# anshium/visual-place-recognition-and-geopose-estimation

Hardware: AMD Instinct MI355X
Metric: images/sec end-to-end (backbone->SALAD->kNN->pose) (higher is better)
Workload: dtype bf16; 1 GPU; DINOv2 vit_large/14 (random init) + SALAD + bf16 kNN k=10 over a 100000-row x 8448 synthetic gallery sharded 1 way(s) + fused (lat,lon,sin,cos) head; 3x224x224 bf16 images; batch_per_gpu=64, global_batch=64, gallery_rows=100000, k=10, parallelism=dp1+gallery-shard1, batches_in_flight=1, graph_retrieval=False

## Files before the change

visual-place-recognition-and-geopose-estimation_amd/csrc/attention.hip:

```cpp
#include <stdlib.h>
#include "vpr_common.h"
#include "vpr_internal.h"

namespace vpr {

constexpr int AT_D = 64;
constexpr int AT_KP = 288;


__device__ __forceinline__ int vtile_off(int row, int chunk) { return row * 128 + ((chunk ^ (row & 7)) << 4); }

struct AttnCtx {
  const char* Ks; const char* Vs; const uint16_t* qb; long long tok_stride; int T, qcol, g, trq, trp;
  float scale_log2e; uint16_t* out; long long out_stride;
  long long row_base, tail_base; int Tp;
};
__device__ __forceinline__ long long attn_row(const AttnCtx& cx, int t) {
  return t < cx.Tp ? cx.row_base + t : cx.tail_base + (t - cx.Tp);
}
typedef __attribute__((ext_vector_type(4))) short s16x4;

__device__ __forceinline__ void attn_load_q(const AttnCtx& cx, int qt, bf16x8 (&bq)[2]) {
  const int qrow = min(qt * 16 + cx.qcol, cx.T - 1);
#pragma unroll
  for (int s = 0; s < 2; ++s)
    bq[s] = *reinterpret_cast<const bf16x8*>(cx.qb + attn_row(cx, qrow) * cx.tok_stride + 32 * s + 8 * cx.g);
}
__device__ __forceinline__ f32x4 attn_qk_block(const AttnCtx& cx, int kb, const bf16x8 (&bq)[2]) {
  f32x4 acc = {0.f, 0.f, 0.f, 0.f};
#pragma unroll
  for (int s = 0; s < 2; ++s)
    acc = __builtin_amdgcn_mfma_f32_16x16x32_bf16(lds_frag(cx.Ks, 16 * kb + cx.qcol, cx.g + 4 * s), bq[s], acc, 0, 0, 0);
  return acc;
}
__device__ __forceinline__ void attn_qk_all(const AttnCtx& cx, const bf16x8 (&bq)[2], f32x4 (&sc)[AT_KP / 16]) {
#pragma unroll
  for (int kb = 0; kb < AT_KP / 16; ++kb) {
    sc[kb] = attn_qk_block(cx, kb, bq);
    if ((kb % 3) == 2) __builtin_amdgcn_sched_barrier(0);
  }
}
__device__ __forceinline__ void attn_mask_block(f32x4& s, int kb, int klast, int lim) {
  if (kb > klast) {
    asm volatile("");
    s = f32x4{-INFINITY, -INFINITY, -INFINITY, -INFINITY};
  } else if (kb == klast) {
    asm volatile("");
#pragma unroll
    for (int e = 0; e < 4; ++e) s[e] = e < lim ? s[e] : -INFINITY;
  }
}
__device__ __forceinline__ float attn_rowmax(const AttnCtx& cx, f32x4 (&sc)[AT_KP / 16]) {
  const int klast = (cx.T - 1) >> 4;
  const int lim = cx.T - 16 * klast - 4 * cx.g;
  if (klast < AT_KP / 16 - 2) {
#pragma unroll
    for (int kb = 0; kb < AT_KP / 16 - 2; ++kb) attn_mask_block(sc[kb], kb, klast, lim);
  }
#pragma unroll
  for (int kb = AT_KP / 16 - 2; kb < AT_KP / 16; ++kb) attn_mask_block(sc[kb], kb, klast, lim);
  float mx = sc[0][0];
#pragma unroll
  for (int kb = 0; kb < AT_KP / 16; ++kb) {
    mx = fmaxf(fmaxf(mx, sc[kb][0]), sc[kb][1]);
    mx = fmaxf(fmaxf(mx, sc[kb][2]), sc[kb][3]);
  }
  mx = fmaxf(mx, __shfl_xor(mx, 16, 64));
  return fmaxf(mx, __shfl_xor(mx, 32, 64));
}
__device__ __forceinline__ void attn_phase1(const AttnCtx& cx, f32x4 (&sc)[AT_KP / 16], float mx,
                                             bf16x8 (&pb)[AT_KP / 32], bool has_next, const bf16x8 (&bq)[2]) {
  const float nm = -mx * cx.scale_log2e;
#pragma unroll
  for (int t = 0; t < AT_KP / 32; ++t) {
    float p[8];
#pragma unroll
    for (int e = 0; e < 4; ++e) {
      p[e] = __builtin_amdgcn_exp2f(fmaf(sc[2 * t][e], cx.scale_log2e, nm));
      p[4 + e] = __builtin_amdgcn_exp2f(fmaf(sc[2 * t + 1][e], cx.scale_log2e, nm));
    }
    if (has_next) {
      sc[2 * t] = attn_qk_block(cx, 2 * t, bq);
      sc[2 * t + 1] = attn_qk_block(cx, 2 * t + 1, bq);
    }
#pragma unroll
    for (int j = 0; j < 8; ++j) pb[t][j] = (__bf16)p[j];
  }
}
__device__ __forceinline__ float attn_phase2(const AttnCtx& cx, const bf16x8 (&pb)[AT_KP / 32], int qt, bool has_next, f32x4 (&sn)[AT_KP / 16]) {
  const bf16x8 ones = {(__bf16)1.f, (__bf16)1.f, (__bf16)1.f, (__bf16)1.f, (__bf16)1.f, (__bf16)1.f, (__bf16)1.f, (__bf16)1.f};
  f32x4 sacc = {0.f, 0.f, 0.f, 0.f};
#pragma unroll
  for (int t = 0; t < AT_KP / 32; ++t) sacc = __builtin_amdgcn_mfma_f32_16x16x32_bf16(ones, pb[t], sacc, 0, 0, 0);
  f32x4 oacc[4];
#pragma unroll
  for (int db = 0; db < 4; ++db) {
    oacc[db] = f32x4{0.f, 0.f, 0.f, 0.f};
#pragma unroll
    for (int t = 0; t < AT_KP / 32; ++t) {
      const int r0 = 32 * t + 4 * cx.g + cx.trq;
      const s16x4 lo = __builtin_amdgcn_ds_read_tr16_b64_v4i16(
          (__attribute__((address_space(3))) s16x4*)(cx.Vs + vtile_off(r0, 2 * db + (cx.trp >> 1)) + 8 * (cx.trp & 1)));
      const s16x4 hi = __builtin_amdgcn_ds_read_tr16_b64_v4i16(
          (__attribute__((address_space(3))) s16x4*)(cx.Vs + vtile_off(r0 + 16, 2 * db + (cx.trp >> 1)) + 8 * (cx.trp & 1)));
      const s16x8 av = {lo[0], lo[1], lo[2], lo[3], hi[0], hi[1], hi[2], hi[3]};
      oacc[db] = __builtin_amdgcn_mfma_f32_16x16x32_bf16(__builtin_bit_cast(bf16x8, av), pb[t], oacc[db], 0, 0, 0);
      if ((t % 3) == 2) __builtin_amdgcn_sched_barrier(0);
    }
  }
  const float inv = 1.0f / sacc[0];
  float mxn = 0.f;
  if (has_next) mxn = attn_rowmax(cx, sn);
  const int q = qt * 16 + cx.qcol;
  if (q < cx.T) {
    uint16_t* orow = cx.out + attn_row(cx, q) * cx.out_stride;
#pragma unroll
    for (int db = 0; db < 4; ++db) {
      ushort4 o;
      o.x = f32_to_bf16_bits(oacc[db][0] * inv);
      o.y = f32_to_bf16_bits(oacc[db][1] * inv);
      o.z = f32_to_bf16_bits(oacc[db][2] * inv);
      o.w = f32_to_bf16_bits(oacc[db][3] * inv);
      *reinterpret_cast<ushort4*>(orow + 16 * db + 4 * cx.g) = o;
    }
  }
  return mxn;
}

template <int NW, bool PIPE, int ABL = 0>
__global__ __launch_bounds__(NW * 64, NW / 2) void attention_kernel(
    const uint16_t* __restrict__ qkv, uint16_t* __restrict__ out, int T, int Tp, long long tail_row0, int H,
    float scale_log2e, int dephase) {
  extern __shared__ __attribute__((aligned(16))) char smem[];
  if (dephase > 0 && blockIdx.x >= 256 && blockIdx.x < 512)
    for (int i = 0; i < dephase; ++i) __builtin_amdgcn_s_sleep(33);
  char* Ks = smem;
  char* Vs = smem + AT_KP * 128;
  const int bh = blockIdx.x, b = bh / H, h = bh % H;
  const int tid = threadIdx.x, lane = tid & 63, wave = tid >> 6;
  const long long tok_stride = 3LL * H * AT_D;
  const uint16_t* qb = qkv + (long long)h * AT_D;
  const uint16_t* kb_ = qb + (long long)H * AT_D;
  const uint16_t* vb = qb + 2LL * H * AT_D;

  constexpr int NT = NW * 64;
  constexpr int AT_MAXT = (AT_KP / 16 + NW - 1) / NW;
  bf16x8 qf[AT_MAXT][2];
  {
    AttnCtx c0;
    c0.qb = qb; c0.tok_stride = tok_stride; c0.T = T; c0.qcol = lane & 15; c0.g = lane >> 4;
    c0.Tp = Tp; c0.row_base = (long long)b * Tp; c0.tail_base = tail_row0 + (long long)b * (T - Tp);
#pragma unroll
    for (int j = 0; j < AT_MAXT; ++j) attn_load_q(c0, min(wave + NW * j, ((T + 15) >> 4) - 1), qf[j]);
  }
  constexpr int NLD = (AT_KP * 8 + NT - 1) / NT;
  s16x8 kreg[NLD], vreg[NLD];
#pragma unroll
  for (int it = 0; it < NLD; ++it) {
    const int i = min(tid + NT * it, AT_KP * 8 - 1);
    const int key = i >> 3, ch = i & 7;
    const int kc = key < T ? key : T - 1;
    const long long krow = kc < Tp ? (long long)b * Tp + kc : tail_row0 + (long long)b * (T - Tp) + (kc - Tp);
    kreg[it] = *reinterpret_cast<const s16x8*>(kb_ + krow * tok_stride + ch * 8);
    vreg[it] = *reinterpret_cast<const s16x8*>(vb + krow * tok_stride + ch * 8);
  }
#pragma unroll
  for (int it = 0; it < NLD; ++it) {
    const int i = min(tid + NT * it, AT_KP * 8 - 1);
    const int key = i >> 3, ch = i & 7;
    const s16x8 z = {0, 0, 0, 0, 0, 0, 0, 0};
    const s16x8 kv = key < T ? kreg[it] : z, vv = key < T ? vreg[it] : z;
    *reinterpret_cast<s16x8*>(Ks + tile_off(key, ch)) = kv;
    *reinterpret_cast<s16x8*>(Vs + vtile_off(key, ch)) = vv;
  }
  __syncthreads();

  if (ABL == 3) return;
  const int qcol = lane & 15, g = lane >> 4;
  const int ntile = (T + 15) >> 4;

  AttnCtx cx;
  cx.Ks = Ks; cx.Vs = Vs; cx.qb = qb; cx.tok_stride = tok_stride; cx.T = T; cx.qcol = qcol; cx.g = g;
  cx.trq = (lane & 15) >> 2; cx.trp = lane & 3; cx.scale_log2e = scale_log2e;
  cx.out = out + (long long)h * AT_D; cx.out_stride = (long long)H * AT_D;
  cx.Tp = Tp; cx.row_base = (long long)b * Tp; cx.tail_base = tail_row0 + (long long)b * (T - Tp);

  f32x4 sc[AT_KP / 16];
  bf16x8 pb[AT_KP / 32];
  if (wave >= ntile) return;
  if constexpr (PIPE) {
    attn_qk_all(cx, qf[0], sc);
    float mx = attn_rowmax(cx, sc);
#pragma unroll
    for (int j = 0; j < AT_MAXT; ++j) {
      const int qt = wave + NW * j;
      if (qt < ntile) {
        const bool has_next = qt + NW < ntile;
        attn_phase1(cx, sc, mx, pb, has_next, qf[j + 1 < AT_MAXT ? j + 1 : j]);
        mx = attn_phase2(cx, pb, qt, has_next, sc);
      }
    }
  } else {
#pragma unroll
    for (int j = 0; j < AT_MAXT; ++j) {
      const int qt = wave + NW * j;
      if (qt < ntile) {
        attn_qk_all(cx, qf[j], sc);
        if (ABL == 4) {
          float a = 0.f;
#pragma unroll
          for (int kb = 0; kb < AT_KP / 16; ++kb) a += sc[kb][0] + sc[kb][1] + sc[kb][2] + sc[kb][3];
          if (qt * 16 + cx.qcol < T) cx.out[attn_row(cx, qt * 16 + cx.qcol) * cx.out_stride + 4 * cx.g] = f32_to_bf16_bits(a);
          continue;
        }
        const float mx = attn_rowmax(cx, sc);
        attn_phase1(cx, sc, mx, pb, false, qf[j]);
        if (ABL == 2) {
          float a = 0.f;
#pragma unroll
          for (int t = 0; t < AT_KP / 32; ++t)
#pragma unroll
            for (int e = 0; e < 8; ++e) a += (float)pb[t][e];
          if (qt * 16 + cx.qcol < T) cx.out[attn_row(cx, qt * 16 + cx.qcol) * cx.out_stride + 4 * cx.g] = f32_to_bf16_bits(a);
          continue;
        }
        attn_phase2(cx, pb, qt, false, sc);
      }
    }
  }
}

constexpr size_t AT_LDS = (size_t)2 * AT_KP * 128;

}

using namespace vpr;

static int attention_launch(const uint16_t* qkv, uint16_t* out, int B, int T, int Tp, long long tail_row0, int H,
                            int head_dim, float scale, void* stream) {
  if (!qkv || !out || B <= 0 || T <= 0 || H <= 0 || Tp < 0 || Tp > T || tail_row0 < 0) return VPR_ERR_INVALID_ARG;
  if (!(scale > 0.f && scale <= 3.4e38f)) return VPR_ERR_INVALID_ARG;
  if (head_dim != AT_D || T > AT_KP || (long long)B * H > 0x7fffffffLL) return VPR_ERR_UNSUPPORTED;
  if ((reinterpret_cast<uintptr_t>(qkv) | reinterpret_cast<uintptr_t>(out)) & 15) return VPR_ERR_UNSUPPORTED;
  const int variant = tune_or(TUNE_ATTN_VARIANT, 0);
  const float c = scale * 1.4426950408889634f;
  const int dephase = (variant >= 20 && variant <= 60) ? variant - 20 : 0;
  hipStream_t st = static_cast<hipStream_t>(stream);
#define VPR_ATTN_LAUNCH(NW, PIPE)                                                                        \
  do {                                                                                                   \
    VPR_TRY_LAUNCH((launch_kernel_lds<attention_kernel<NW, PIPE>>(dim3((unsigned)(B * H)), dim3(NW * 64), AT_LDS, st, \
                                                                  qkv, out, T, Tp, tail_row0, H, c, dephase)));     \
  } while (0)
#ifdef VPR_ABLATION
#define VPR_ATTN_ABL(A)                                                                                   \
  do {                                                                                                   \
    VPR_TRY_LAUNCH((launch_kernel_lds<attention_kernel<8, false, A>>(dim3((unsigned)(B * H)), dim3(512), AT_LDS, st, \
                                                                     qkv, out, T, Tp, tail_row0, H, c, 0)));        \
  } while (0)
#endif
  switch (variant) {
    case 1: VPR_ATTN_LAUNCH(4, false); break;
    case 2: VPR_ATTN_LAUNCH(4, true); break;
    case 3: VPR_ATTN_LAUNCH(6, false); break;
#ifdef VPR_ABLATION
    case 12: VPR_ATTN_ABL(2); break;
    case 13: VPR_ATTN_ABL(3); break;
    case 14: VPR_ATTN_ABL(4); break;
#endif
    default: VPR_ATTN_LAUNCH(8, false); break;
  }
#undef VPR_ATTN_LAUNCH
#ifdef VPR_ABLATION
#undef VPR_ATTN_ABL
#endif
  return VPR_OK;
}

extern "C" int vpr_attention_qkv_bf16(const uint16_t* qkv, uint16_t* out, int B, int T, int H, int head_dim,
                                      float scale, void* stream) {
  return attention_launch(qkv, out, B, T, T, 0, H, head_dim, scale, stream);
}

extern "C" int vpr_attention_qkv_split_bf16(const uint16_t* qkv, uint16_t* out, int B, int T, int body_tokens,
                                            long long tail_row0, int H, int head_dim, float scale, void* stream) {
  return attention_launch(qkv, out, B, T, body_tokens, tail_row0, H, head_dim, scale, stream);
}
```

visual-place-recognition-and-geopose-estimation_amd/csrc/backbone_rows.h:

```cpp
#pragma once
#include <initializer_list>
#include "vpr_common.h"
#include "vpr_internal.h"

namespace vpr {


template <int NCH>
__device__ __forceinline__ void ln_load_row(const uint16_t* x, const uint16_t* res, uint16_t* sum_out, const float* pre_bias,
                                            long long off, bool store_sum, int nchunks, int lane, float (&v)[NCH][8], float& s) {
  s = 0.f;
#pragma unroll
  for (int i = 0; i < NCH; ++i) {
    const int ch = lane + 64 * i;
    if (ch < nchunks) {
      const s16x8 q = *reinterpret_cast<const s16x8*>(x + off + ch * 8);
      if (res != nullptr) {
        const s16x8 r = *reinterpret_cast<const s16x8*>(res + off + ch * 8);
        s16x8 o;
#pragma unroll
        for (int e = 0; e < 8; ++e) {
          const uint16_t sb = f32_to_bf16_bits(bf16_bits_to_f32((uint16_t)q[e]) + bf16_bits_to_f32((uint16_t)r[e]));
          o[e] = (short)sb;
          v[i][e] = bf16_bits_to_f32(sb);
          s += v[i][e];
        }
        if (store_sum) *reinterpret_cast<s16x8*>(sum_out + off + ch * 8) = o;
      } else if (pre_bias != nullptr) {
        const float4 p0 = *reinterpret_cast<const float4*>(pre_bias + ch * 8);
        const float4 p1 = *reinterpret_cast<const float4*>(pre_bias + ch * 8 + 4);
        const float pb[8] = {p0.x, p0.y, p0.z, p0.w, p1.x, p1.y, p1.z, p1.w};
#pragma unroll
        for (int e = 0; e < 8; ++e) { v[i][e] = bf16_bits_to_f32((uint16_t)q[e]) + pb[e]; s += v[i][e]; }
      } else {
#pragma unroll
        for (int e = 0; e < 8; ++e) { v[i][e] = bf16_bits_to_f32((uint16_t)q[e]); s += v[i][e]; }
      }
    } else {
#pragma unroll
      for (int e = 0; e < 8; ++e) v[i][e] = 0.f;
    }
  }
}

template <int NCH>
__device__ __forceinline__ void ln_stats(const float (&v)[NCH][8], float s, int C, float eps, int lane, float& mean, float& rstd) {
  mean = wave_sum(s) / (float)C;
  float ss = 0.f;
#pragma unroll
  for (int i = 0; i < NCH; ++i)
    if (lane + 64 * i < (C >> 3)) {
#pragma unroll
      for (int e = 0; e < 8; ++e) { const float d = v[i][e] - mean; ss = fmaf(d, d, ss); }
    }
  rstd = 1.0f / sqrtf(wave_sum(ss) / (float)C + eps);
}

template <typename ParamT>
__device__ __forceinline__ float ln_param(const ParamT* p, int ch, int e) {
  if constexpr (sizeof(ParamT) == 16) return bf16_bits_to_f32((uint16_t)p[ch][e]);
  else if constexpr (sizeof(ParamT) == 2) return bf16_bits_to_f32((uint16_t)p[ch * 8 + e]);
  else return p[ch * 8 + e];
}

template <int NCH, typename ParamT>
__device__ __forceinline__ void ln_store_row(const float (&v)[NCH][8], float mean, float rstd, const ParamT* gamma,
                                             const ParamT* beta, uint16_t* y, long long off, int nchunks, int lane) {
#pragma unroll
  for (int i = 0; i < NCH; ++i) {
    const int ch = lane + 64 * i;
    if (ch < nchunks) {
      s16x8 o;
#pragma unroll
      for (int e = 0; e < 8; ++e) {
        const float g = ln_param(gamma, ch, e), b = ln_param(beta, ch, e);
        o[e] = (short)f32_to_bf16_bits((v[i][e] - mean) * rstd * g + b);
      }
      *reinterpret_cast<s16x8*>(y + off + ch * 8) = o;
    }
  }
}


template <int MBW, bool QUAD = false>
struct SkinnyOperands {
  const uint16_t* wp;
  const uint16_t* ip[MBW];
  __device__ __forceinline__ SkinnyOperands(const uint16_t* W, int ldw, int n0, int N, const uint16_t* in, long long ldi, int m0,
                                            int M, int lane) {
    const int r = QUAD ? lane >> 2 : lane & 15, g = QUAD ? lane & 3 : lane >> 4;
    wp = W + (long long)min(n0 + r, N - 1) * ldw + 8 * g;
#pragma unroll
    for (int mb = 0; mb < MBW; ++mb) ip[mb] = in + (long long)min(m0 + mb * 16 + r, M - 1) * ldi + 8 * g;
  }
};

__device__ __forceinline__ bf16x8 skinny_to_mfma_lane(bf16x8 f) {
  typedef __attribute__((ext_vector_type(4))) int i32x4;
  const int src = 4 * (4 * (int)(threadIdx.x & 15) + (int)((threadIdx.x & 63) >> 4));
  i32x4 v = __builtin_bit_cast(i32x4, f);
#pragma unroll
  for (int e = 0; e < 4; ++e) v[e] = __builtin_amdgcn_ds_bpermute(src, v[e]);
  return __builtin_bit_cast(bf16x8, v);
}

template <int UNR, int MBW, bool QUAD>
__device__ __forceinline__ void skinny_k_slice(const SkinnyOperands<MBW, QUAD>& o, int kbeg, int kend, f32x4 (&acc)[MBW]) {
  const auto frag = [](const uint16_t* p) -> bf16x8 {
    const bf16x8 f = *reinterpret_cast<const bf16x8*>(p);
    if constexpr (QUAD) return skinny_to_mfma_lane(f); else return f;
  };
  f32x4 a[MBW];
#pragma unroll
  for (int mb = 0; mb < MBW; ++mb) a[mb] = f32x4{0.f, 0.f, 0.f, 0.f};
  int ks = kbeg;
  for (; ks + UNR <= kend; ks += UNR) {
    bf16x8 wf[UNR], xf[UNR][MBW];
#pragma unroll
    for (int u = 0; u < UNR; ++u) {
      wf[u] = frag(o.wp + (ks + u) * 32);
#pragma unroll
      for (int mb = 0; mb < MBW; ++mb) xf[u][mb] = frag(o.ip[mb] + (ks + u) * 32);
    }
#pragma unroll
    for (int u = 0; u < UNR; ++u)
#pragma unroll
      for (int mb = 0; mb < MBW; ++mb) a[mb] = __builtin_amdgcn_mfma_f32_16x16x32_bf16(wf[u], xf[u][mb], a[mb], 0, 0, 0);
  }
  for (; ks < kend; ++ks) {
    const bf16x8 wf = frag(o.wp + ks * 32);
#pragma unroll
    for (int mb = 0; mb < MBW; ++mb)
      a[mb] = __builtin_amdgcn_mfma_f32_16x16x32_bf16(wf, frag(o.ip[mb] + ks * 32), a[mb], 0, 0, 0);
  }
#pragma unroll
  for (int mb = 0; mb < MBW; ++mb) acc[mb] = a[mb];
}

template <int NW, int MBW>
__device__ __forceinline__ bool skinny_reduce(const f32x4 (&acc)[MBW], float (&red)[NW][MBW][64][4], int lane, int wave, f32x4& s) {
#pragma unroll
  for (int mb = 0; mb < MBW; ++mb) *reinterpret_cast<f32x4*>(&red[wave][mb][lane][0]) = acc[mb];
  __syncthreads();
  if (NW > MBW && wave >= MBW) return false;
  s = *reinterpret_cast<const f32x4*>(&red[0][wave][lane][0]);
#pragma unroll
  for (int p = 1; p < NW; ++p) {
    const f32x4 t = *reinterpret_cast<const f32x4*>(&red[p][wave][lane][0]);
    s[0] += t[0]; s[1] += t[1]; s[2] += t[2]; s[3] += t[3];
  }
  return true;
}

__device__ __forceinline__ void skinny_store4(uint16_t* op, const uint16_t (&ob)[4], int n, int N, int ldo) {
  if (n + 3 < N && (ldo & 3) == 0) {
    ushort4 o;
    o.x = ob[0]; o.y = ob[1]; o.z = ob[2]; o.w = ob[3];
    *reinterpret_cast<ushort4*>(op) = o;
  } else {
    for (int e = 0; e < 4 && n + e < N; ++e) op[e] = ob[e];
  }
}

__device__ __forceinline__ float gelu_tanh(float x) {
  const float u = 0.7978845608028654f * x * fmaf(0.044715f * x, x, 1.0f);
  return x / (1.0f + __expf(-2.0f * u));
}


__device__ __forceinline__ void row_stats_write16(float* __restrict__ row_stats, int p, int m, int M, const uint16_t (&ob)[4],
                                                  const float* __restrict__ stats_bias, int n, int N, int lane) {
  float t[4];
#pragma unroll
  for (int e = 0; e < 4; ++e)
    t[e] = bf16_bits_to_f32(ob[e]) + (stats_bias != nullptr && n + e < N ? stats_bias[n + e] : 0.f);
  float sm = (t[0] + t[1]) + (t[2] + t[3]);
  sm += __shfl_xor(sm, 16, 64);
  sm += __shfl_xor(sm, 32, 64);
  const float mean = sm * (1.0f / 16.0f);
  float m2 = 0.f;
#pragma unroll
  for (int e = 0; e < 4; ++e) { const float d = t[e] - mean; m2 = fmaf(d, d, m2); }
  m2 += __shfl_xor(m2, 16, 64);
  m2 += __shfl_xor(m2, 32, 64);
  if ((lane >> 4) == 0 && m < M) {
    float* dst = row_stats + ((long long)p * M + m) * 2;
    dst[0] = mean; dst[1] = m2;
  }
}

__device__ __forceinline__ void row_stats_merge(const float* __restrict__ row_stats, int P, int M, int row, int part, float& mean,
                                                float& m2) {
  const float* ps = row_stats + (long long)row * 2;
  const long long pstride = (long long)M * 2;
  float sm = 0.f;
#pragma unroll 8
  for (int p = part; p < P; p += 4) sm += ps[p * pstride];
  sm += __shfl_xor(sm, 1, 64);
  sm += __shfl_xor(sm, 2, 64);
  mean = sm / (float)P;
  m2 = 0.f;
#pragma unroll 8
  for (int p = part; p < P; p += 4) {
    const float2 q = *reinterpret_cast<const float2*>(ps + p * pstride);
    const float d = q.x - mean;
    m2 += q.y + 16.0f * d * d;
  }
  m2 += __shfl_xor(m2, 1, 64);
  m2 += __shfl_xor(m2, 2, 64);
}

inline bool ln_shape_ok(long long M, int C) { return (C % 8) == 0 && C <= 2048 && M <= 0x1fffffffcLL; }

inline int ln_check(std::initializer_list<const void*> chunked, const void* gamma, const void* beta, long long M, int C) {
  for (const void* p : chunked)
    if (!p) return VPR_ERR_INVALID_ARG;
  if (!gamma || !beta || M < 0 || C <= 0) return VPR_ERR_INVALID_ARG;
  if (M == 0) return VPR_OK;
  if (!ln_shape_ok(M, C)) return VPR_ERR_UNSUPPORTED;
  for (const void* p : chunked)
    if (!aligned16(p)) return VPR_ERR_UNSUPPORTED;
  return VPR_OK;
}

template <typename F>
inline int ln_dispatch_nch(int C, F&& f) {
  switch ((C / 8 + 63) / 64) {
    case 1: return f(std::integral_constant<int, 1>{});
    case 2: return f(std::integral_constant<int, 2>{});
    case 3: return f(std::integral_constant<int, 3>{});
    case 4: return f(std::integral_constant<int, 4>{});
    default: return VPR_ERR_UNSUPPORTED;
  }
}

}
```

visual-place-recognition-and-geopose-estimation_amd/csrc/layernorm.hip:

```cpp
#include "backbone_rows.h"

namespace vpr {

template <int NCH, typename ParamT, int RW>
__global__ __launch_bounds__(256) void layernorm_bf16_kernel(
    const uint16_t* __restrict__ x, const uint16_t* __restrict__ res, uint16_t* __restrict__ sum_out,
    const float* __restrict__ pre_bias, const ParamT* __restrict__ gamma, const ParamT* __restrict__ beta,
    float eps, uint16_t* __restrict__ y, long long M, int C) {
  static_assert(RW == 1 || RW == 2, "one or two rows per wave");
  const int lane = threadIdx.x & 63, wave = threadIdx.x >> 6;
  const long long row0 = ((long long)blockIdx.x * 4 + wave) * RW;
  if (row0 >= M) return;
  const int nchunks = C >> 3;
  const bool second = RW == 2 && row0 + 1 < M;
  float v[RW][NCH][8], s[RW], mean, rstd;
  ln_load_row<NCH>(x, res, sum_out, pre_bias, row0 * C, true, nchunks, lane, v[0], s[0]);
  if constexpr (RW == 2)
    ln_load_row<NCH>(x, res, sum_out, pre_bias, (second ? row0 + 1 : M - 1) * C, second, nchunks, lane, v[1], s[1]);
  ln_stats<NCH>(v[0], s[0], C, eps, lane, mean, rstd);
  ln_store_row<NCH>(v[0], mean, rstd, gamma, beta, y, row0 * C, nchunks, lane);
  if constexpr (RW == 2) {
    if (!second) return;
    ln_stats<NCH>(v[1], s[1], C, eps, lane, mean, rstd);
    ln_store_row<NCH>(v[1], mean, rstd, gamma, beta, y, (row0 + 1) * C, nchunks, lane);
  }
}

template <typename ParamT>
static int launch_ln(const uint16_t* x, const uint16_t* res, uint16_t* sum_out, const float* pb, const ParamT* g, const ParamT* b,
                     float eps, uint16_t* y, long long M, int C, hipStream_t stream) {
  const int rw = tune_or(TUNE_LN_ROWS, 1);
  return ln_dispatch_nch(C, [&](auto nch) {
    constexpr int NCH = decltype(nch)::value;
    if constexpr (NCH <= 2)
      if (rw == 2)
        return launch_kernel(layernorm_bf16_kernel<NCH, ParamT, 2>, dim3((unsigned)((M + 7) / 8)), dim3(256), 0, stream,
                             x, res, sum_out, pb, g, b, eps, y, M, C);
    return launch_kernel(layernorm_bf16_kernel<NCH, ParamT, 1>, dim3((unsigned)((M + 3) / 4)), dim3(256), 0, stream,
                         x, res, sum_out, pb, g, b, eps, y, M, C);
  });
}

static int ln_entry(std::initializer_list<const void*> chunked, const uint16_t* x, const uint16_t* res, uint16_t* sum_out,
                    const float* pb, const void* gamma, const void* beta, int params_are_bf16, float eps, uint16_t* y,
                    long long M, int C, void* stream) {
  const int st = ln_check(chunked, gamma, beta, M, C);
  if (st != VPR_OK || M == 0) return st;
  hipStream_t s = static_cast<hipStream_t>(stream);
  if (params_are_bf16)
    return launch_ln(x, res, sum_out, pb, static_cast<const uint16_t*>(gamma), static_cast<const uint16_t*>(beta), eps, y, M, C, s);
  return launch_ln(x, res, sum_out, pb, static_cast<const float*>(gamma), static_cast<const float*>(beta), eps, y, M, C, s);
}

}

using namespace vpr;

extern "C" int vpr_layernorm_bf16(const uint16_t* x, const void* gamma, const void* beta, int params_are_bf16,
                                  float eps, uint16_t* y, long long M, int C, void* stream) {
  return ln_entry({x, y}, x, nullptr, nullptr, nullptr, gamma, beta, params_are_bf16, eps, y, M, C, stream);
}

extern "C" int vpr_add_layernorm_bf16(const uint16_t* x, const uint16_t* res, uint16_t* sum_out, const void* gamma,
                                      const void* beta, int params_are_bf16, float eps, uint16_t* y, long long M,
                                      int C, void* stream) {
  return ln_entry({x, y, res, sum_out}, x, res, sum_out, nullptr, gamma, beta, params_are_bf16, eps, y, M, C, stream);
}

extern "C" int vpr_bias_layernorm_bf16(const uint16_t* x, const float* pre_bias, const void* gamma, const void* beta,
                                       int params_are_bf16, float eps, uint16_t* y, long long M, int C, void* stream) {
  return ln_entry({x, y, pre_bias}, x, nullptr, nullptr, pre_bias, gamma, beta, params_are_bf16, eps, y, M, C, stream);
}
```

visual-place-recognition-and-geopose-estimation_amd/csrc/vpr_common.h:

```cpp
#pragma once
#include <hip/hip_runtime.h>
#include <stdint.h>

namespace vpr {

typedef __attribute__((ext_vector_type(8))) short s16x8;
typedef __attribute__((ext_vector_type(8))) __bf16 bf16x8;
typedef __attribute__((ext_vector_type(4))) float f32x4;
typedef __attribute__((ext_vector_type(16))) float f32x16;
typedef __attribute__((ext_vector_type(4))) int i32x4;
typedef __attribute__((ext_vector_type(8))) int i32x8;

constexpr int WAVE = 64;

__device__ __forceinline__ long long vpr_clock_now() {
  unsigned long long t;
  asm volatile("s_memrealtime %0\n\ts_waitcnt lgkmcnt(0)" : "=s"(t) : : "memory");
  return (long long)t;
}

__device__ __forceinline__ float bf16_bits_to_f32(uint16_t v) {
  return __uint_as_float(((uint32_t)v) << 16);
}
__device__ __forceinline__ uint16_t f32_to_bf16_bits(float f) {
  __bf16 h = (__bf16)f;
  return __builtin_bit_cast(uint16_t, h);
}

__device__ __forceinline__ void split_hi_lo(float v, uint16_t& hi, uint16_t& lo) {
  hi = f32_to_bf16_bits(v);
  lo = f32_to_bf16_bits(v - bf16_bits_to_f32(hi));
}

__device__ __forceinline__ void lds_barrier() {
  asm volatile("s_waitcnt lgkmcnt(0)" ::: "memory");
  __builtin_amdgcn_s_barrier();
}

__device__ __forceinline__ float wave_sum(float v) {
#pragma unroll
  for (int o = 32; o > 0; o >>= 1) v += __shfl_xor(v, o, 64);
  return v;
}
__device__ __forceinline__ float wave_max(float v) {
#pragma unroll
  for (int o = 32; o > 0; o >>= 1) v = fmaxf(v, __shfl_xor(v, o, 64));
  return v;
}
__device__ __forceinline__ double wave_sum_f64(double v) {
#pragma unroll
  for (int o = 32; o > 0; o >>= 1) v += __shfl_xor(v, o, 64);
  return v;
}

template <int CTRL>
__device__ __forceinline__ float dpp_f32(float v) {
  return __builtin_bit_cast(float, __builtin_amdgcn_update_dpp(0, __builtin_bit_cast(int, v), CTRL, 0xf, 0xf, true));
}
__device__ __forceinline__ float row16_max(float v) {
  v = fmaxf(v, dpp_f32<0xB1>(v));
  v = fmaxf(v, dpp_f32<0x4E>(v));
  v = fmaxf(v, dpp_f32<0x141>(v));
  v = fmaxf(v, dpp_f32<0x140>(v));
  return v;
}
__device__ __forceinline__ float row16_sum(float v) {
  v += dpp_f32<0xB1>(v);
  v += dpp_f32<0x4E>(v);
  v += dpp_f32<0x141>(v);
  v += dpp_f32<0x140>(v);
  return v;
}

__device__ __forceinline__ uint32_t f32_orderable(float f) {
  const uint32_t u = __float_as_uint(f);
  return (u & 0x80000000u) ? ~u : (u | 0x80000000u);
}
__device__ __forceinline__ float f32_from_orderable(uint32_t o) {
  const uint32_t u = (o & 0x80000000u) ? (o & 0x7fffffffu) : ~o;
  return __uint_as_float(u);
}
__device__ __forceinline__ unsigned long long make_key(float v, int idx) {
  return ((unsigned long long)f32_orderable(v) << 32) | (uint32_t)(0x7fffffff - idx);
}
__device__ __forceinline__ int key_idx(unsigned long long k) { return 0x7fffffff - (int)(uint32_t)k; }
__device__ __forceinline__ float key_val(unsigned long long k) { return f32_from_orderable((uint32_t)(k >> 32)); }

constexpr unsigned long long KEY_DEAD = 0ull;

__device__ __forceinline__ unsigned long long candidate_key(float val, int id, bool in_range) {
  return (in_range && id >= 0) ? make_key(val, id) : KEY_DEAD;
}
__device__ __forceinline__ void store_entry(unsigned long long k, float* __restrict__ out_val,
                                            int32_t* __restrict__ out_idx, long long o, int index_base = 0) {
  out_val[o] = k == KEY_DEAD ? -INFINITY : key_val(k);
  out_idx[o] = k == KEY_DEAD ? -1 : key_idx(k) + index_base;
}

constexpr int TILE_ROW_BYTES = 128;
__device__ __forceinline__ int tile_off(int row, int chunk) {
  return row * TILE_ROW_BYTES + ((chunk ^ ((row >> 1) & 7)) << 4);
}
__device__ __forceinline__ int stage_src_off(int tr, int lane) {
  return ((lane & 7) ^ ((tr >> 1) & 7)) << 4;
}

template <int AUX = 0>
__device__ __forceinline__ void glds16(const void* gsrc, void* lds_wave_base) {
  __builtin_amdgcn_global_load_lds(
      (const __attribute__((address_space(1))) void*)gsrc,
      (__attribute__((address_space(3))) void*)lds_wave_base, 16, 0, AUX);
}

__device__ __forceinline__ bf16x8 lds_frag(const char* tile, int row, int chunk) {
  return *reinterpret_cast<const bf16x8*>(tile + tile_off(row, chunk));
}

template <typename Chunk>
__device__ __forceinline__ i32x8 e4m3_operand(Chunk lo, Chunk hi) {
  const i32x4 l = __builtin_bit_cast(i32x4, lo), h = __builtin_bit_cast(i32x4, hi);
  return i32x8{l[0], l[1], l[2], l[3], h[0], h[1], h[2], h[3]};
}
constexpr int E8M0_ONE = 127;
__device__ __forceinline__ f32x4 mfma_e4m3_16x16x128(i32x8 a, i32x8 b, f32x4 c) {
  return __builtin_amdgcn_mfma_scale_f32_16x16x128_f8f6f4(a, b, c, 0, 0, 0, E8M0_ONE, 0, E8M0_ONE);
}
__device__ __forceinline__ f32x16 mfma_e4m3_32x32x64(i32x8 a, i32x8 b, f32x16 c) {
  return __builtin_amdgcn_mfma_scale_f32_32x32x64_f8f6f4(a, b, c, 0, 0, 0, E8M0_ONE, 0, E8M0_ONE);
}

__device__ __forceinline__ int xcd_tile(int orig, int nwg) {
  const int xcd = orig & 7, q = nwg >> 3, r = nwg & 7;
  return (xcd < r ? xcd * (q + 1) : r * (q + 1) + (xcd - r) * q) + (orig >> 3);
}

__device__ __forceinline__ uint4 philox4x32_10(uint4 c, uint32_t k0, uint32_t k1) {
#pragma unroll
  for (int r = 0; r < 10; ++r) {
    const uint32_t hi0 = __umulhi(0xD2511F53u, c.x), lo0 = 0xD2511F53u * c.x;
    const uint32_t hi1 = __umulhi(0xCD9E8D57u, c.z), lo1 = 0xCD9E8D57u * c.z;
    c = make_uint4(hi1 ^ c.y ^ k0, lo1, hi0 ^ c.w ^ k1, lo0);
    k0 += 0x9E3779B9u;
    k1 += 0xBB67AE85u;
  }
  return c;
}

struct SlabRowMajor {
  float* part; int B, hidden;
  __device__ __forceinline__ float* at(int slice, int b, int h) const { return part + ((long long)slice * B + b) * hidden + h; }
  __device__ __forceinline__ long long slice_stride() const { return (long long)B * hidden; }
};
struct SlabTiles {
  float* part; int mtiles, ntiles;
  __device__ __forceinline__ float* at(int slice, int b, int h) const {
    return part + (((long long)slice * mtiles + (b >> 6)) * ntiles + (h >> 6)) * 4096 + (b & 63) * 64 + (h & 63);
  }
  __device__ __forceinline__ long long slice_stride() const { return (long long)mtiles * ntiles * 4096; }
};

template <int CH, int STRIDE>
__device__ __forceinline__ void mfma_f32_slice(const float4* xa, const float4* wa, const float4* wb, int first, int s_begin,
                                               int s_end, f32x4& acc0, f32x4& acc1) {
  for (int base = s_begin; base < s_end; base += STRIDE * CH) {
    float4 a[CH], w0[CH], w1[CH];
#pragma unroll
    for (int i = 0; i < CH; ++i) {
      const int s = min(base + first + STRIDE * i, s_end - 1);
      a[i] = xa[s * 4];
      w0[i] = wa[s * 4];
      w1[i] = wb[s * 4];
    }
#pragma unroll
    for (int i = 0; i < CH; ++i) {
      if (base + first + STRIDE * i < s_end) {
        acc0 = __builtin_amdgcn_mfma_f32_16x16x4f32(a[i].x, w0[i].x, acc0, 0, 0, 0);
        acc1 = __builtin_amdgcn_mfma_f32_16x16x4f32(a[i].x, w1[i].x, acc1, 0, 0, 0);
        acc0 = __builtin_amdgcn_mfma_f32_16x16x4f32(a[i].y, w0[i].y, acc0, 0, 0, 0);
        acc1 = __builtin_amdgcn_mfma_f32_16x16x4f32(a[i].y, w1[i].y, acc1, 0, 0, 0);
        acc0 = __builtin_amdgcn_mfma_f32_16x16x4f32(a[i].z, w0[i].z, acc0, 0, 0, 0);
        acc1 = __builtin_amdgcn_mfma_f32_16x16x4f32(a[i].z, w1[i].z, acc1, 0, 0, 0);
        acc0 = __builtin_amdgcn_mfma_f32_16x16x4f32(a[i].w, w0[i].w, acc0, 0, 0, 0);
        acc1 = __builtin_amdgcn_mfma_f32_16x16x4f32(a[i].w, w1[i].w, acc1, 0, 0, 0);
      }
    }
  }
}

__device__ __forceinline__ void mfma_f32_store_rows(const SlabRowMajor& slab, int slice, int b0, int h0, int lane,
                                                    const f32x4& acc0, const f32x4& acc1) {
  const int r = lane & 15, kg = lane >> 4;
#pragma unroll
  for (int e = 0; e < 4; ++e) {
    const int b = b0 + 4 * kg + e;
    if (b < slab.B) {
      float* p = slab.at(slice, b, h0);
      p[r] = acc0[e];
      p[16 + r] = acc1[e];
    }
  }
}

__device__ __forceinline__ float bf16_lo(uint32_t w) { return __uint_as_float(w << 16); }
__device__ __forceinline__ float bf16_hi(uint32_t w) { return __uint_as_float(w & 0xffff0000u); }
__device__ __forceinline__ uint2 pack_bf16x4(f32x4 v) {
  uint2 h;
  h.x = (uint32_t)f32_to_bf16_bits(v[0]) | ((uint32_t)f32_to_bf16_bits(v[1]) << 16);
  h.y = (uint32_t)f32_to_bf16_bits(v[2]) | ((uint32_t)f32_to_bf16_bits(v[3]) << 16);
  return h;
}

__device__ __forceinline__ bool shard_row(int id, int n_local, int index_base, long long& r) {
  r = (long long)id - index_base;
  return r >= 0 && r < n_local;
}

constexpr int ORDER_MAX_KC = 128;
constexpr unsigned long long KEY_NAN_HI = 1ull << 32;
__device__ __forceinline__ int order_rank(const float* __restrict__ scores, const int32_t* __restrict__ idx, long long b, int kc,
                                          int n_local, int index_base, unsigned long long* s_key, float& val, int& id) {
  const int j = threadIdx.x;
  unsigned long long key = KEY_DEAD;
  val = -INFINITY;
  id = -1;
  if (j < kc) {
    const int cand = idx[b * kc + j];
    long long r;
    if (shard_row(cand, n_local, index_base, r)) {
      const float s = scores[b * kc + j];
      id = cand;
      if (isnan(s)) key = KEY_NAN_HI | (uint32_t)(0x7fffffff - cand);
      else { key = make_key(s, cand); val = s; }
    }
  }
  s_key[j] = key;
  __syncthreads();
  if (j >= kc) return -1;
  int rank = 0;
  for (int i = 0; i < kc; ++i) {
    const unsigned long long o = s_key[i];
    rank += (o > key || (o == key && i < j)) ? 1 : 0;
  }
  return rank;
}

template <int NWAVES>
__device__ __forceinline__ float block_sum_in_wave_order(float wave_total, float* s_part, int lane, int wave) {
  if (lane == 0) s_part[wave] = wave_total;
  __syncthreads();
  float s = 0.f;
#pragma unroll
  for (int w = 0; w < NWAVES; ++w) s += s_part[w];
  return s;
}
__device__ __forceinline__ bool norm_unusable(float n2) { return !(n2 > 0.f) || isinf(n2); }

}
```

Measured before the change: 5691 images/s.

## Add persistent streaming LayerNorm kernel with prefetch and VALU wave reduction

Adds a grid-stride persistent LayerNorm kernel sized to resident waves per CU. It prefetches the next row while reducing and storing the current one, and holds gamma/beta in registers across rows. It also adds a wave sum built from permlane swaps plus DPP, meant to avoid LDS/shuffle latency, and makes the streaming kernel the default path. The attention dephase range now uses the actual CU count instead of a hardcoded 256. The cost is higher register pressure, since parameters and the prefetched row stay live, and reliance on gfx950 permlane builtins.

```diff
diff --git a/visual-place-recognition-and-geopose-estimation_amd/csrc/attention.hip b/visual-place-recognition-and-geopose-estimation_amd/csrc/attention.hip
--- a/visual-place-recognition-and-geopose-estimation_amd/csrc/attention.hip
+++ b/visual-place-recognition-and-geopose-estimation_amd/csrc/attention.hip
@@ -130,9 +130,9 @@
 template <int NW, bool PIPE, int ABL = 0>
 __global__ __launch_bounds__(NW * 64, NW / 2) void attention_kernel(
     const uint16_t* __restrict__ qkv, uint16_t* __restrict__ out, int T, int Tp, long long tail_row0, int H,
-    float scale_log2e, int dephase) {
+    float scale_log2e, int dephase, int cus) {
   extern __shared__ __attribute__((aligned(16))) char smem[];
-  if (dephase > 0 && blockIdx.x >= 256 && blockIdx.x < 512)
+  if (dephase > 0 && (int)blockIdx.x >= cus && (int)blockIdx.x < 2 * cus)
     for (int i = 0; i < dephase; ++i) __builtin_amdgcn_s_sleep(33);
   char* Ks = smem;
   char* Vs = smem + AT_KP * 128;
@@ -245,17 +245,18 @@
   const int variant = tune_or(TUNE_ATTN_VARIANT, 0);
   const float c = scale * 1.4426950408889634f;
   const int dephase = (variant >= 20 && variant <= 60) ? variant - 20 : 0;
+  const int cus = device_cu_count() > 0 ? device_cu_count() : 1;
   hipStream_t st = static_cast<hipStream_t>(stream);
 #define VPR_ATTN_LAUNCH(NW, PIPE)                                                                        \
   do {                                                                                                   \
     VPR_TRY_LAUNCH((launch_kernel_lds<attention_kernel<NW, PIPE>>(dim3((unsigned)(B * H)), dim3(NW * 64), AT_LDS, st, \
-                                                                  qkv, out, T, Tp, tail_row0, H, c, dephase)));     \
+                                                                  qkv, out, T, Tp, tail_row0, H, c, dephase, cus)));     \
   } while (0)
 #ifdef VPR_ABLATION
 #define VPR_ATTN_ABL(A)                                                                                   \
   do {                                                                                                   \
     VPR_TRY_LAUNCH((launch_kernel_lds<attention_kernel<8, false, A>>(dim3((unsigned)(B * H)), dim3(512), AT_LDS, st, \
-                                                                     qkv, out, T, Tp, tail_row0, H, c, 0)));        \
+                                                                     qkv, out, T, Tp, tail_row0, H, c, 0, cus)));        \
   } while (0)
 #endif
   switch (variant) {
diff --git a/visual-place-recognition-and-geopose-estimation_amd/csrc/backbone_rows.h b/visual-place-recognition-and-geopose-estimation_amd/csrc/backbone_rows.h
--- a/visual-place-recognition-and-geopose-estimation_amd/csrc/backbone_rows.h
+++ b/visual-place-recognition-and-geopose-estimation_amd/csrc/backbone_rows.h
@@ -44,8 +44,61 @@
 }
 
 template <int NCH>
+__device__ __forceinline__ void ln_fetch_row(const uint16_t* x, const uint16_t* res, long long off, int nchunks, int lane,
+                                             s16x8 (&q)[NCH], s16x8 (&r)[NCH]) {
+#pragma unroll
+  for (int i = 0; i < NCH; ++i) {
+    const int ch = lane + 64 * i;
+    if (ch < nchunks) {
+      q[i] = *reinterpret_cast<const s16x8*>(x + off + ch * 8);
+      if (res != nullptr) r[i] = *reinterpret_cast<const s16x8*>(res + off + ch * 8);
+    }
+  }
+}
+
+__device__ __forceinline__ void ln_pre_bias_chunk(const float* pre_bias, int ch, float (&pb)[8]) {
+  const float4 p0 = *reinterpret_cast<const float4*>(pre_bias + ch * 8);
+  const float4 p1 = *reinterpret_cast<const float4*>(pre_bias + ch * 8 + 4);
+  pb[0] = p0.x; pb[1] = p0.y; pb[2] = p0.z; pb[3] = p0.w; pb[4] = p1.x; pb[5] = p1.y; pb[6] = p1.z; pb[7] = p1.w;
+}
+
+template <int NCH>
+__device__ __forceinline__ void ln_widen_row(const s16x8 (&q)[NCH], const s16x8 (&r)[NCH], bool has_res, uint16_t* sum_out,
+                                             long long off, bool has_pb, const float (&pb)[NCH][8], int nchunks, int lane,
+                                             float (&v)[NCH][8], float& s) {
+  s = 0.f;
+#pragma unroll
+  for (int i = 0; i < NCH; ++i) {
+    const int ch = lane + 64 * i;
+    if (ch < nchunks) {
+      if (has_res) {
+        s16x8 o;
+#pragma unroll
+        for (int e = 0; e < 8; ++e) {
+          const uint16_t sb = f32_to_bf16_bits(bf16_bits_to_f32((uint16_t)q[i][e]) + bf16_bits_to_f32((uint16_t)r[i][e]));
+          o[e] = (short)sb;
+          v[i][e] = bf16_bits_to_f32(sb);
+          s += v[i][e];
+        }
+        *reinterpret_cast<s16x8*>(sum_out + off + ch * 8) = o;
+      } else if (has_pb) {
+#pragma unroll
+        for (int e = 0; e < 8; ++e) { v[i][e] = bf16_bits_to_f32((uint16_t)q[i][e]) + pb[i][e]; s += v[i][e]; }
+      } else {
+#pragma unroll
+        for (int e = 0; e < 8; ++e) { v[i][e] = bf16_bits_to_f32((uint16_t)q[i][e]); s += v[i][e]; }
+      }
+    } else {
+#pragma unroll
+      for (int e = 0; e < 8; ++e) v[i][e] = 0.f;
+    }
+  }
+}
+
+template <int NCH, bool SHFL = false>
 __device__ __forceinline__ void ln_stats(const float (&v)[NCH][8], float s, int C, float eps, int lane, float& mean, float& rstd) {
-  mean = wave_sum(s) / (float)C;
+  const auto lanes_sum = [](float t) { if constexpr (SHFL) return wave_sum(t); else return wave_sum_valu(t); };
+  mean = lanes_sum(s) / (float)C;
   float ss = 0.f;
 #pragma unroll
   for (int i = 0; i < NCH; ++i)
@@ -53,7 +106,7 @@
 #pragma unroll
       for (int e = 0; e < 8; ++e) { const float d = v[i][e] - mean; ss = fmaf(d, d, ss); }
     }
-  rstd = 1.0f / sqrtf(wave_sum(ss) / (float)C + eps);
+  rstd = 1.0f / sqrtf(lanes_sum(ss) / (float)C + eps);
 }
 
 template <typename ParamT>
@@ -63,6 +116,10 @@
   else return p[ch * 8 + e];
 }
 
+__device__ __forceinline__ uint16_t ln_norm_bits(float v, float mean, float rstd, float g, float b) {
+  return f32_to_bf16_bits((v - mean) * rstd * g + b);
+}
+
 template <int NCH, typename ParamT>
 __device__ __forceinline__ void ln_store_row(const float (&v)[NCH][8], float mean, float rstd, const ParamT* gamma,
                                              const ParamT* beta, uint16_t* y, long long off, int nchunks, int lane) {
@@ -74,8 +131,39 @@
 #pragma unroll
       for (int e = 0; e < 8; ++e) {
         const float g = ln_param(gamma, ch, e), b = ln_param(beta, ch, e);
-        o[e] = (short)f32_to_bf16_bits((v[i][e] - mean) * rstd * g + b);
+        o[e] = (short)ln_norm_bits(v[i][e], mean, rstd, g, b);
       }
+      *reinterpret_cast<s16x8*>(y + off + ch * 8) = o;
+    }
+  }
+}
+
+template <int NCH>
+struct LnHeldParams {
+  float g[NCH][8], b[NCH][8];
+  template <typename ParamT>
+  __device__ __forceinline__ void fetch(const ParamT* gamma, const ParamT* beta, int nchunks, int lane) {
+#pragma unroll
+    for (int i = 0; i < NCH; ++i) {
+      const int ch = lane + 64 * i;
+      if (ch < nchunks) {
+#pragma unroll
+        for (int e = 0; e < 8; ++e) { g[i][e] = ln_param(gamma, ch, e); b[i][e] = ln_param(beta, ch, e); }
+      }
+    }
+  }
+};
+
+template <int NCH>
+__device__ __forceinline__ void ln_store_row_held(const float (&v)[NCH][8], float mean, float rstd, const LnHeldParams<NCH>& p,
+                                                  uint16_t* y, long long off, int nchunks, int lane) {
+#pragma unroll
+  for (int i = 0; i < NCH; ++i) {
+    const int ch = lane + 64 * i;
+    if (ch < nchunks) {
+      s16x8 o;
+#pragma unroll
+      for (int e = 0; e < 8; ++e) o[e] = (short)ln_norm_bits(v[i][e], mean, rstd, p.g[i][e], p.b[i][e]);
       *reinterpret_cast<s16x8*>(y + off + ch * 8) = o;
     }
   }
@@ -223,6 +311,12 @@
   return VPR_OK;
 }
 
+constexpr int ln_stream_waves_per_cu(int nch) { return nch <= 1 ? 32 : nch == 2 ? 20 : nch == 3 ? 16 : 12; }
+inline unsigned ln_stream_blocks(long long M, int cus, int nch) {
+  const long long resident = (long long)(cus > 0 ? cus : 1) * (ln_stream_waves_per_cu(nch) / 4), needed = (M + 3) / 4;
+  return (unsigned)(needed < resident ? needed : resident);
+}
+
 template <typename F>
 inline int ln_dispatch_nch(int C, F&& f) {
   switch ((C / 8 + 63) / 64) {
diff --git a/visual-place-recognition-and-geopose-estimation_amd/csrc/layernorm.hip b/visual-place-recognition-and-geopose-estimation_amd/csrc/layernorm.hip
--- a/visual-place-recognition-and-geopose-estimation_amd/csrc/layernorm.hip
+++ b/visual-place-recognition-and-geopose-estimation_amd/csrc/layernorm.hip
@@ -17,21 +17,105 @@
   ln_load_row<NCH>(x, res, sum_out, pre_bias, row0 * C, true, nchunks, lane, v[0], s[0]);
   if constexpr (RW == 2)
     ln_load_row<NCH>(x, res, sum_out, pre_bias, (second ? row0 + 1 : M - 1) * C, second, nchunks, lane, v[1], s[1]);
-  ln_stats<NCH>(v[0], s[0], C, eps, lane, mean, rstd);
+  ln_stats<NCH, true>(v[0], s[0], C, eps, lane, mean, rstd);
   ln_store_row<NCH>(v[0], mean, rstd, gamma, beta, y, row0 * C, nchunks, lane);
   if constexpr (RW == 2) {
     if (!second) return;
-    ln_stats<NCH>(v[1], s[1], C, eps, lane, mean, rstd);
+    ln_stats<NCH, true>(v[1], s[1], C, eps, lane, mean, rstd);
     ln_store_row<NCH>(v[1], mean, rstd, gamma, beta, y, (row0 + 1) * C, nchunks, lane);
   }
 }
 
+template <int NCH, typename ParamT, int FORM>
+__global__ __launch_bounds__(256, ln_stream_waves_per_cu(NCH) / 4) void layernorm_stream_kernel(
+    const uint16_t* __restrict__ x, const uint16_t* __restrict__ res_, uint16_t* __restrict__ sum_out,
+    const float* __restrict__ pre_bias, const ParamT* __restrict__ gamma, const ParamT* __restrict__ beta,
+    float eps, uint16_t* __restrict__ y, long long M, int C) {
+  const int lane = threadIdx.x & 63, wave = __builtin_amdgcn_readfirstlane(threadIdx.x >> 6);
+  const long long W = (long long)gridDim.x * 4;
+  long long row = (long long)blockIdx.x * 4 + wave;
+  if (row >= M) return;
+  const int nchunks = C >> 3;
+  const uint16_t* res = FORM == 1 ? res_ : nullptr;
+  s16x8 q[NCH], r[NCH];
+  float pb[NCH][8];
+  LnHeldParams<NCH> p;
+  ln_fetch_row<NCH>(x, res, row * C, nchunks, lane, q, r);
+  if constexpr (FORM == 2) {
+#pragma unroll
+    for (int i = 0; i < NCH; ++i)
+      if (lane + 64 * i < nchunks) ln_pre_bias_chunk(pre_bias, lane + 64 * i, pb[i]);
+  }
+  p.fetch(gamma, beta, nchunks, lane);
+  for (;;) {
+    float v[NCH][8], s, mean, rstd;
+    ln_widen_row<NCH>(q, r, FORM == 1, sum_out, row * C, FORM == 2, pb, nchunks, lane, v, s);
+    const long long next = row + W;
+    if (next < M) ln_fetch_row<NCH>(x, res, next * C, nchunks, lane, q, r);
+    ln_stats<NCH>(v, s, C, eps, lane, mean, rstd);
+    ln_store_row_held<NCH>(v, mean, rstd, p, y, row * C, nchunks, lane);
+    if (next >= M) return;
+    row = next;
+  }
+}
+
+#ifdef VPR_ABLATION
+template <int NCH, int ABL>
+__global__ __launch_bounds__(256) void layernorm_ablation_kernel(const uint16_t* __restrict__ x, float eps, uint16_t* __restrict__ y,
+                                                                 long long M, int C) {
+  const int lane = threadIdx.x & 63, wave = threadIdx.x >> 6;
+  const long long row = (long long)blockIdx.x * 4 + wave;
+  if (row >= M) return;
+  const int nchunks = C >> 3;
+  s16x8 q[NCH], r[NCH];
+  float v[NCH][8], s = 0.f, ss = 0.f, mean, rstd;
+  ln_fetch_row<NCH>(x, nullptr, row * C, nchunks, lane, q, r);
+#pragma unroll
+  for (int i = 0; i < NCH; ++i)
+#pragma unroll
+    for (int e = 0; e < 8; ++e) { v[i][e] = lane + 64 * i < nchunks ? bf16_bits_to_f32((uint16_t)q[i][e]) + 0.25f : 0.f; s += v[i][e]; }
+  if constexpr (ABL == 1) {
+    ln_stats<NCH, true>(v, s, C, eps, lane, mean, rstd);
+  } else {
+    mean = s / (float)C;
+#pragma unroll
+    for (int i = 0; i < NCH; ++i)
+#pragma unroll
+      for (int e = 0; e < 8; ++e) { const float d = v[i][e] - mean; ss = fmaf(d, d, ss); }
+    rstd = 1.0f / sqrtf(ss / (float)C + eps);
+  }
+#pragma unroll
+  for (int i = 0; i < NCH; ++i) {
+    const int ch = lane + 64 * i;
+    if (ch < nchunks) {
+      s16x8 o;
+#pragma unroll
+      for (int e = 0; e < 8; ++e) o[e] = (short)ln_norm_bits(v[i][e], mean, rstd, 1.25f, 0.5f);
+      *reinterpret_cast<s16x8*>(y + row * C + ch * 8) = o;
+    }
+  }
+}
+#endif
+
 template <typename ParamT>
 static int launch_ln(const uint16_t* x, const uint16_t* res, uint16_t* sum_out, const float* pb, const ParamT* g, const ParamT* b,
                      float eps, uint16_t* y, long long M, int C, hipStream_t stream) {
-  const int rw = tune_or(TUNE_LN_ROWS, 1);
+  const int rw = tune_or(TUNE_LN_ROWS, 0);
   return ln_dispatch_nch(C, [&](auto nch) {
     constexpr int NCH = decltype(nch)::value;
+#ifdef VPR_ABLATION
+    if ((rw == 11 || rw == 12) && pb != nullptr)
+      return launch_kernel(rw == 11 ? layernorm_ablation_kernel<NCH, 1> : layernorm_ablation_kernel<NCH, 2>, dim3((unsigned)((M + 3) / 4)),
+                           dim3(256), 0, stream, x, eps, y, M, C);
+#endif
+    if (rw != 1 && rw != 2) {
+      const dim3 grid(ln_stream_blocks(M, device_cu_count(), NCH));
+      if (res != nullptr)
+        return launch_kernel(layernorm_stream_kernel<NCH, ParamT, 1>, grid, dim3(256), 0, stream, x, res, sum_out, pb, g, b, eps, y, M, C);
+      if (pb != nullptr)
+        return launch_kernel(layernorm_stream_kernel<NCH, ParamT, 2>, grid, dim3(256), 0, stream, x, res, sum_out, pb, g, b, eps, y, M, C);
+      return launch_kernel(layernorm_stream_kernel<NCH, ParamT, 0>, grid, dim3(256), 0, stream, x, res, sum_out, pb, g, b, eps, y, M, C);
+    }
     if constexpr (NCH <= 2)
       if (rw == 2)
         return launch_kernel(layernorm_bf16_kernel<NCH, ParamT, 2>, dim3((unsigned)((M + 7) / 8)), dim3(256), 0, stream,
diff --git a/visual-place-recognition-and-geopose-estimation_amd/csrc/vpr_common.h b/visual-place-recognition-and-geopose-estimation_amd/csrc/vpr_common.h
--- a/visual-place-recognition-and-geopose-estimation_amd/csrc/vpr_common.h
+++ b/visual-place-recognition-and-geopose-estimation_amd/csrc/vpr_common.h
@@ -69,6 +69,24 @@
   v += dpp_f32<0x4E>(v);
   v += dpp_f32<0x141>(v);
   v += dpp_f32<0x140>(v);
+  return v;
+}
+
+__device__ __forceinline__ float wave_sum_valu(float v) {
+  {
+    const unsigned u = __float_as_uint(v);
+    const auto r = __builtin_amdgcn_permlane32_swap(u, u, false, false);
+    v = __uint_as_float(r[0]) + __uint_as_float(r[1]);
+  }
+  {
+    const unsigned u = __float_as_uint(v);
+    const auto r = __builtin_amdgcn_permlane16_swap(u, u, false, false);
+    v = __uint_as_float(r[0]) + __uint_as_float(r[1]);
+  }
+  v += dpp_f32<0x128>(v);
+  v += dpp_f32<0x1B>(dpp_f32<0x141>(v));
+  v += dpp_f32<0x4E>(v);
+  v += dpp_f32<0xB1>(v);
   return v;
 }
 
```

Result: no change. 5727 images/s (median of 6 runs) (+0.6%).
